# safes/RayTracing-Weekend

Hardware: AMD Instinct MI355X
Metric: Msamples/s, Cornell box 1920x1080 4096spp (higher is better)
Workload: dtype f32

## Files before the change

### raytracing_weekend_amd/csrc/rtw_hip.hip

```cpp
#include <hip/hip_runtime.h>

#include <algorithm>
#include <cmath>
#include <cstdio>
#include <cstdlib>
#include <cstring>
#include <condition_variable>
#include <exception>
#include <mutex>
#include <new>
#include <stdexcept>
#include <string>
#include <thread>
#include <vector>

#include "../../include/rtw.h"
#include "rtw_bvh.h"
#include "rtw_device.h"
#include "rtw_plan.h"
#include "rtw_kernels.h"
#include "rtw_guides.h"
#include "rtw_adaptive.h"
#ifndef RTW_SPLIT_BUILD
#include "rtw_guides.hip"
// ... 795 lines not shown
    }
    const unsigned pix_grid = pixel_grid(c, npix);
    for (const PathPass& ps : plan.passes) {
        HIP_TRY(c, hipMemsetAsync(c->d_queue, 0, 4, s));
        HIP_TRY(c, hipMemsetAsync(c->d_queue + 4, 0, 4, s));
        hipEvent_t ev_a = nullptr, ev_b = nullptr;
        HIP_TRY(c, log.event(ev_a));
        HIP_TRY(c, log.event(ev_b));
        HIP_TRY(c, hipEventRecord(ev_a, s));
        CallLog::Timed tp;
        HIP_TRY(c, log.open(tp, RTW_K_PATH, s));
        for (int part = 0; part < 2; part++) {
            const PathLaunch& l = ps.part[part];
            if (l.count == 0) continue;
            KArgs a = base;
            a.stats = c->d_stats;
            a.sample0 = (uint32_t)P->sample_offset;
            a.queue = c->d_queue + (part == 0 ? 0 : 4);
            a.order = c->d_order;
            a.order_counts = c->d_queue + 1;
            a.blocksum = c->blocksum + (part == 0 ? 0 : ps.slots_coarse) * npix;
            a.unit_sums = (part == 0 && plan.unit_sums) ? 1u : 0u;
            a.n_jobs = (uint32_t)l.n_jobs; a.n_ranges = (uint32_t)l.n_ranges; a.units_per_job = (uint32_t)l.jb;
            a.block0 = (uint32_t)(ps.b0 + l.first); a.n_blocks_pass = (uint32_t)l.count; a.unit_blocks = (uint32_t)l.unit_blocks;
            hipStream_t ls = part == 0 ? s : c->stream2;
            if (part == 1) HIP_TRY(c, hipStreamWaitEvent(ls, ev_a, 0));
            launch(RTW_K_PATH, P->rng_kind, a, l.grid, 0, ls);
            log.launches++;
            if (part == 1) {
                HIP_TRY(c, hipEventRecord(ev_b, ls));
                HIP_TRY(c, hipStreamWaitEvent(s, ev_b, 0));
            }
        }
        HIP_TRY(c, log.close(tp, s));
        if (plan.unit_sums)
            hipLaunchKernelGGL(k_resolve_blocks, dim3(pix_grid), dim3(kBlock), 0, s, (const float4*)c->blocksum, c->accum, (uint32_t)npix, (uint32_t)ps.slots_coarse,
                               (uint32_t)(ps.nb - ps.nb_coarse), (uint32_t)(ps.b0 + ps.nb_coarse));
        else
            hipLaunchKernelGGL(k_resolve_blocks, dim3(pix_grid), dim3(kBlock), 0, s, (const float4*)c->blocksum, c->accum, (uint32_t)npix, 0u, (uint32_t)ps.nb, (uint32_t)ps.b0);
    }
    hipLaunchKernelGGL(k_finish, dim3(pix_grid), dim3(kBlock), 0, s, (const float4*)c->accum, (const float4*)nullptr, (const float4*)nullptr, out, (uint32_t)npix, (float)P->spp);
    return RTW_OK;
}

int issue_batch(rtw_ctx* c, const WavefrontPlan& w, const Tuning& tune, KArgs a, rtw_ctx::Lane& L, size_t paths, size_t Sb, hipEvent_t ready,
                CallLog& log, bool list) {
    const size_t lds = c->lds_bytes;
    const uint32_t regions = w.grid_for(paths);
    HIP_TRY(c, hipStreamWaitEvent(L.st, ready, 0));
    HIP_TRY(c, hipMemsetAsync(L.cnt, 0, (size_t)regions * (w.sched.size() + 2) * sizeof(uint32_t), L.st));
    a.lbuf = L.lbuf;
    a.stats = c->d_stats;
    a.n_regions = regions;
    a.n_paths = (uint32_t)paths;
    a.region_cap = (uint32_t)w.cap_for(paths);
    a.trace_first = w.split_first ? 1u : 0u;
    a.first_group_log2 = 0;
    while (a.first_group_log2 < (uint32_t)tune.first_group_log2 && (Sb >> (a.first_group_log2 + 1)) << (a.first_group_log2 + 1) == Sb) a.first_group_log2++;
    int cur = 0;
    size_t ci = 0;
    a.out = L.buf[0];
    a.hit_out = L.hit[0];
    a.cnt_out = L.cnt;
    a.depth = 0; a.n_iter = 1;
    log.launches++;
    HIP_TRY(c, log.launch(L.st, RTW_K_FIRST, a, (int)regions, c->sc.use_bvh ? (size_t)(kBlock / 64) * (size_t)c->stack_depth * sizeof(uint32_t) : 0, kBlock, list));
    for (const Step& st : w.sched) {
        a.in = L.buf[cur];
        a.hit = L.hit[cur];
        a.hit_out = L.hit[cur];
        a.cnt_in = L.cnt + ci * regions;
        a.depth = (uint32_t)st.depth;
        a.n_iter = (uint32_t)st.n_iter;
        if (st.kind == RTW_K_TRACE) {
            if (c->sc.use_bvh) {
                KArgs at = a;
                at.sc.n_lds_nodes = w.trace_nodes; at.sc.n_lds_leaves = w.trace_leaves;
                HIP_TRY(c, log.launch(L.st, RTW_K_TRACE, at, w.trace_grid, w.trace_lds, w.trace_block));
            } else {
                HIP_TRY(c, log.launch(L.st, RTW_K_TRACE, a, (int)regions, lds));
            }
        } else {
            a.out = L.buf[cur ^ 1];
            a.hit_out = L.hit[cur ^ 1];
            a.cnt_out = L.cnt + (ci + 1) * regions;
            HIP_TRY(c, log.launch(L.st, st.kind, a, (int)regions, st.kind == RTW_K_BOUNCE ? lds : 0));
            cur ^= 1;
            ci++;
        }
        log.launches++;
    }
    return RTW_OK;
}

int render_wavefront(rtw_ctx* c, const rtw_params* P, const Tuning& tune, const KArgs& base, float4* out, hipStream_t s, CallLog& log) {
    const size_t npix = base.npix;
    const SceneFacts sf{c->sc.use_bvh != 0, c->sc.n_vol, c->n_tree_nodes, c->n_tree_leaves, c->stack_depth, c->sc.stack_wide != 0};
    WavefrontPlan w;
    for (;;) {
        w = plan_wavefront(tune, npix, P->spp, P->samples_per_pass, P->max_depth, c->pool_cap, c->n_cu, sf);
        if (w.trace_lds > 48 * 1024) {
            DScene ts = c->sc;
            ts.n_lds_nodes = w.trace_nodes;
            const void* f = (const void*)trace_bvh_kernel(w.trace_block, trace_bvh_mode(ts));
            HIP_TRY(c, hipFuncSetAttribute(f, hipFuncAttributeMaxDynamicSharedMemorySize, (int)w.trace_lds));
        }
        const int rc = ensure_pool(c, w.n_lanes, (size_t)w.regions_max * w.region_cap_max, npix, w.cnt_words, c->sc.n_lights > 0);
        if (rc == RTW_OK) break;
        if (rc != RTW_ERR_OOM || P->samples_per_pass > 0 || w.S <= 1) return rc;
        free_pool(c);
        (void)hipGetLastError();
        c->pool_cap = std::max<size_t>((size_t)tune.lanes * npix, npix * w.S * (size_t)tune.lanes / 2);
    }

    HIP_TRY(c, hipEventRecord(log.begin, s));
    HIP_TRY(c, hipMemsetAsync(c->accum, 0, npix * sizeof(float4), s));
    HIP_TRY(c, hipMemsetAsync(c->part, 0, npix * sizeof(float4), s));
    HIP_TRY(c, hipMemsetAsync(c->upart, 0, npix * sizeof(float4), s));
    HIP_TRY(c, hipMemsetAsync(c->d_stats, 0, (kStatRows + 1) * 8 * sizeof(unsigned long long), s));
    const unsigned pix_grid = pixel_grid(c, npix);
    hipEvent_t ev_ready = nullptr;
    if (P->max_depth > 0) {
        HIP_TRY(c, log.event(ev_ready));
        HIP_TRY(c, hipEventRecord(ev_ready, s));
    }
    for (size_t s0 = 0, b = 0; P->max_depth > 0 && s0 < (size_t)P->spp; b++) {
        const size_t Sb = w.batch_size(b, s0);
        rtw_ctx::Lane& L = c->lane[b % (size_t)w.n_lanes];
        KArgs a = base;
        a.sample0 = (uint32_t)(P->sample_offset + (int)s0);
        const int rc = issue_batch(c, w, tune, a, L, npix * Sb, Sb, b < (size_t)w.n_lanes ? ev_ready : L.ev_free, log, false);
        if (rc) return rc;
        HIP_TRY(c, hipEventRecord(L.ev_done, L.st));
        HIP_TRY(c, hipStreamWaitEvent(s, L.ev_done, 0));
        hipLaunchKernelGGL(k_resolve, dim3(pix_grid), dim3(kBlock), 0, s, (const float4*)L.lbuf, c->accum, c->upart, c->part, (uint32_t)npix, (uint32_t)Sb, (uint32_t)s0);
        HIP_TRY(c, hipEventRecord(L.ev_free, s));
        s0 += Sb;
    }
    hipLaunchKernelGGL(k_finish, dim3(pix_grid), dim3(kBlock), 0, s, (const float4*)c->accum, (const float4*)c->upart, (const float4*)c->part, out, (uint32_t)npix, (float)P->spp);
    return RTW_OK;
}

int print_diagnostics(rtw_ctx* c, bool path, const unsigned long long* hs) {
#ifdef RTW_PHASE_TIMERS
    if (path) {
        unsigned long long ph[8];
        HIP_TRY(c, hipMemcpy(ph, c->d_stats + kStatRows * 8, sizeof ph, hipMemcpyDeviceToHost));
        double tot = 0;
        for (int q = 0; q < 6; q++) tot += (double)ph[q];
        const char* nm[6] = {"refill", "regen", "walk_r", "shade_a", "walk_s", "shade_b"};
        fprintf(stderr, "[rtw] k_path wave-cycles by phase:");
        for (int q = 0; q < 6; q++) fprintf(stderr, " %s %.1f%%", nm[q], 100.0 * (double)ph[q] / tot);
        fprintf(stderr, " (total %.3g wave-cycles, %.0f per 64 segments)\n", tot, tot / ((double)hs[0] / 64.0));
    }
#endif
#ifdef RTW_SUBPHASE_TIMERS
    if (path) {
        static std::vector<unsigned long long> tab((size_t)kSubWaves * kSubRows);
        HIP_TRY(c, hipMemcpyFromSymbol(tab.data(), HIP_SYMBOL(g_sub_cyc), tab.size() * sizeof(unsigned long long)));
        double sum[kSubRows] = {0};
        for (size_t w = 0; w < (size_t)kSubWaves; w++) for (int q = 0; q < 14; q++) sum[q] += (double)tab[w * kSubRows + q];
        double tot = 0;
        for (int q = 0; q < 14; q++) tot += sum[q];
        const char* nm[9] = {"outside", "hitrec+philox", "lambert", "light", "metal", "diel", "iso", "nee", "entry"};
        fprintf(stderr, "[rtw] k_path wave-cycles by sub-phase of the closest-hit program:");
        for (int q = 0; q < 9; q++) fprintf(stderr, " %s %.1f%%", nm[q], 100.0 * sum[q] / tot);
        fprintf(stderr, " (total %.3g)\n", tot);
        std::fill(tab.begin(), tab.end(), 0ull);
        HIP_TRY(c, hipMemcpyToSymbol(HIP_SYMBOL(g_sub_cyc), tab.data(), tab.size() * sizeof(unsigned long long)));
    }
#endif
#ifdef RTW_TRACE_COUNT
    {
        unsigned long long w[7];
        HIP_TRY(c, hipMemcpy(w, c->d_stats + kStatRows * 8, sizeof w, hipMemcpyDeviceToHost));
        const double rays = (double)w[6];
        fprintf(stderr, "[rtw] k_trace_bvh: rays %.4g; per ray: node visits %.2f, primitive tests %.2f; wave steps per 64 rays: inner %.2f (lanes busy %.2f), leaf %.2f (lanes busy %.2f), outer %.2f\n",
                rays, (double)hs[6] / rays, (double)hs[7] / rays, (double)w[0] * 64.0 / rays, (double)hs[6] / ((double)w[0] * 64.0), (double)w[1] * 64.0 / rays,
                (double)hs[7] / ((double)w[1] * 64.0), (double)hs[2 + RTW_K_BOUNCE] * 64.0 / rays);
        const double tt = (double)(w[2] + w[3] + w[4] + w[5]);
        fprintf(stderr, "[rtw] k_trace_bvh wave-cycles: refill %.1f%% inner %.1f%% leaf %.1f%% finish %.1f%% (%.0f per 64 rays; per inner wave step %.0f, per leaf wave step %.0f)\n",
                100.0 * (double)w[2] / tt, 100.0 * (double)w[3] / tt, 100.0 * (double)w[4] / tt, 100.0 * (double)w[5] / tt, tt * 64.0 / rays,
                (double)w[3] / (double)w[0], (double)w[4] / (double)w[1]);
    }
#endif
    (void)c; (void)path; (void)hs;
    return RTW_OK;
}

KArgs render_args(const rtw_ctx* c, const rtw_params* P, size_t npix) {
    KArgs base = shard_args(c->sc, P, npix);
    if (P->estimator != RTW_EST_REFERENCE) {
        base.sc.estimator = P->estimator; base.sc.has_tex = P->estimator == RTW_EST_MIXTURE ? 2 : 1;
        base.sc.ray_tmin = 1.0e-3f; base.sc.probe_eps = 1.0e-3f;
    }
    return base;
}
bool path_pipeline(const rtw_ctx* c, const rtw_params* P, const Tuning& tune) {
    const bool path_small = !c->sc.use_bvh && c->sc.n_prims <= kPathMaxPrims && (c->sc.n_walk_words > 0 || c->sc.has_tex);
    const bool fits16 = P->width <= 65535 && P->height <= 65535;
    return P->max_depth > 0 && tune.path != 0 && fits16 && path_small;
}

int render_single(rtw_ctx* c, const rtw_params* P, void* d_rgba, hipStream_t s, rtw_stats* stats) {
    HIP_TRY(c, hipSetDevice(c->device));
    if (!s) s = c->stream;
    const size_t npix = shard_rows(P) * (size_t)P->width;
    if (stats) memset(stats, 0, sizeof *stats);
    if (npix == 0) return RTW_OK;
    if (npix > 0xffffffffull / 2) return fail(c, RTW_ERR_UNSUPPORTED, "tile too large");

    const Tuning tune = read_tuning();
    CallLog log{c, P->rng_kind, stats != nullptr && tune.kernel_timing};
    HIP_TRY(c, log.event(log.begin));
    HIP_TRY(c, log.event(log.end));
    const KArgs base = render_args(c, P, npix);
    const bool use_path = path_pipeline(c, P, tune);
    int rc = use_path ? render_path(c, P, tune, base, (float4*)d_rgba, s, log) : render_wavefront(c, P, tune, base, (float4*)d_rgba, s, log);
    if (rc) return rc;
    HIP_TRY(c, hipGetLastError());
    HIP_TRY(c, hipEventRecord(log.end, s));
    HIP_TRY(c, hipEventSynchronize(log.end));

    unsigned long long hs[8] = {0, 0, 0, 0, 0, 0, 0, 0};
    {
        unsigned long long rows_[kStatRows * 8];
        HIP_TRY(c, hipMemcpy(rows_, c->d_stats, sizeof rows_, hipMemcpyDeviceToHost));
        for (uint32_t r = 0; r < kStatRows; r++)
            for (int k = 0; k < 8; k++) hs[k] += rows_[r * 8 + k];
    }
    rc = print_diagnostics(c, use_path, hs);
    if (rc) return rc;
    if (stats) {
        float ms = 0.f;
        HIP_TRY(c, hipEventElapsedTime(&ms, log.begin, log.end));
        stats->seconds = (double)ms * 1e-3;
        stats->bounce_seconds = stats->seconds;
        for (const CallLog::Timed& t : log.timed) {
            float m = 0.f;
            HIP_TRY(c, hipEventElapsedTime(&m, t.a, t.b));
            stats->kernel_seconds[t.kind] += (double)m * 1e-3;
            stats->kernel_launches[t.kind]++;
        }
        for (int k = 0; k < RTW_K_COUNT; k++) stats->kernel_segments[k] = hs[2 + k];
        stats->bounce_launches = log.launches;
        stats->samples = (uint64_t)npix * (uint64_t)P->spp;
        stats->segments = hs[0];
        stats->shadow_rays = hs[1];
        stats->algorithmic_bytes = 128ull * stats->segments + 32ull * stats->samples;
    }
    return RTW_OK;
}

__global__ void __launch_bounds__(256) k_interleave(const float4* __restrict__ stage, float4* __restrict__ out, uint32_t width, uint32_t rows, uint32_t n,
                                                    const uint32_t* __restrict__ shard_off) {
    const size_t total = (size_t)rows * width;
    for (size_t i = (size_t)blockIdx.x * blockDim.x + threadIdx.x; i < total; i += (size_t)gridDim.x * blockDim.x) {
        const uint32_t r = (uint32_t)(i / width), x = (uint32_t)(i - (size_t)r * width);
        const uint32_t g = r % n, l = r / n;
        out[i] = stage[((size_t)shard_off[g] + l) * width + x];
    }
}

int run_shard(rtw_ctx* kc, Worker& w) {
    test_fault("worker");
    if (hipSetDevice(kc->device) != hipSuccess) return fail(kc, RTW_ERR_DEVICE, "hipSetDevice failed");
    if (w.npix == 0) return RTW_OK;
    if (w.npix > kc->out_pix) {
        if (kc->d_out) (void)hipFree(kc->d_out);
        kc->d_out = nullptr; kc->out_pix = 0;
        if (hipMalloc(&kc->d_out, w.npix * sizeof(float4)) != hipSuccess) return fail(kc, RTW_ERR_OOM, "shard buffer");
        kc->out_pix = w.npix;
    }
    const int rc = render_single(kc, &w.P, kc->d_out, nullptr, w.want_stats ? &w.st : nullptr);
    if (rc) return rc;
    HIP_TRY(kc, hipMemcpyPeerAsync(w.gather_dst, w.gather_dev, kc->d_out, kc->device, w.npix * sizeof(float4), kc->stream));
    HIP_TRY(kc, hipStreamSynchronize(kc->stream));
    return RTW_OK;
}
void worker_main(rtw_ctx* kc) {
    Worker& w = *kc->worker;
    for (;;) {
        try {
            std::unique_lock<std::mutex> lk(w.m);
            w.cv.wait(lk, [&] { return w.has_job || w.quit; });
            if (w.quit) return;
            lk.unlock();
            int rc;
            try {
                rc = run_shard(kc, w);
            } catch (const std::bad_alloc&) {
                rc = fail_nothrow(kc, RTW_ERR_OOM, "out of host memory in a worker thread (std::bad_alloc)");
            } catch (const std::exception& e) {
                rc = fail_nothrow(kc, RTW_ERR_DEVICE, e.what());
            } catch (...) {
                rc = fail_nothrow(kc, RTW_ERR_DEVICE, "unknown exception in a worker thread");
            }
            lk.lock();
            w.rc = rc; w.has_job = false; w.done = true;
            lk.unlock();
            w.cv.notify_all();
        } catch (...) {
            w.rc = RTW_ERR_DEVICE; w.has_job = false; w.done = true;
            w.cv.notify_all();
            return;
        }
// ... 551 lines not shown
```

### raytracing_weekend_amd/csrc/rtw_kernels.h

```cpp
#pragma once
#include "rtw_device.h"
#include "rtw_plan.h"

namespace rtwk {
using namespace rtwdev;

#ifndef RTW_MIN_WAVES
#define RTW_MIN_WAVES 1
#endif
#ifdef RTW_SUBPHASE_TIMERS
constexpr int kSubRows = 16, kSubWaves = 8192;
__device__ unsigned long long g_sub_cyc[kSubWaves][kSubRows];
RTW_DEV constexpr int rtw_sub_id(const char* n) {
    return n[0] != 's' || n[1] != 'a' ? 0 : n[3] == 'h' ? 1 : n[3] == 'l' && n[4] == 'a' ? 2 : n[3] == 'l' ? 3 : n[3] == 'm' ? 4 : n[3] == 'd' ? 5 : n[3] == 'i' ? 6 : n[3] == 'n' ? 7 : 0;
}
RTW_DEV void rtw_sub_stamp(int id) {
    const unsigned long long t_in = __builtin_amdgcn_s_memtime();
    if ((threadIdx.x & 63u) == 0u) {
        unsigned long long* row = g_sub_cyc[(blockIdx.x * (blockDim.x >> 6) + (threadIdx.x >> 6)) % kSubWaves];
        const unsigned long long open_id = row[14], t0 = row[15];
        if (t0 != 0ull) row[open_id] += t_in - t0;
        row[14] = (unsigned long long)id;
        __builtin_amdgcn_s_waitcnt(0);
        row[15] = __builtin_amdgcn_s_memtime();
// ... 983 lines not shown
                        fogged = volume_pass<Rng<KIND>, true>(A.sc, so, nee.dir, nee.tmin, 0.0f, gt, g, tv, pv);
                    }
                    if (fogged) nee.has = false;
                    else { p.ldir = nee.dir; p.ltmax = nee.tmax; p.c = vmul(nee.rad, p.T); }
                }
                const bool alive = shade_b<KIND>(A.depth, A.max_depth, g, ev, so, sd, att, radiance, p.o, p.d, p.T, p.L, TEX == 2 && A.sc.estimator == RTW_EST_MIXTURE);
                if (ev == EV_HIT) p.o = so;
                p.a = g.a; p.b = g.b;
                if (alive) {
                    p.ray_time = (KIND == RTW_RNG_TEA_LCG || A.sc.has_motion) ? g.ray_time(A.depth + 1u) : 0.0f;
                    p.b = g.b;
                    keep = true;
                } else if (nee.has) {
                    p.gk |= kZombie;
                    keep = true;
                } else {
                    finish_path(A, path_id_of<KIND>(A, p), p.L);
                }
            }
        }
        compact_store(A, s_cursor, keep, p);
    }
    cursor_publish(A, s_cursor, n_seg, n_shadow, RTW_K_SHADE);
}

template <int KIND, int TEX>
__global__ void __launch_bounds__(kBlock, RTW_MIN_WAVES) k_bounce(const KArgs A) {
    extern __shared__ uint32_t s_stack[];
    RTW_WORKLIST_SHARED
    RTW_CURSOR_SHARED
    RTW_NOISE_SHARED
    const uint32_t tid = threadIdx.x;
    cursor_init(s_cursor);
    const uint32_t* noise_lds = stage_noise<(TEX != 0)>(A.sc, s_noise);
    const TravMem tm = trav_mem(A.sc, s_stack, kBlock, tid);
    uint32_t n_seg = 0, n_shadow = 0;
    const WorkList wl = worklist_init(A.cnt_in, A.n_regions, s_pref, s_part);
    for (uint32_t vc = blockIdx.x; vc < wl.total_chunks; vc += gridDim.x) {
        uint32_t region, chunk, n_valid;
        worklist_lookup(wl, A.n_regions, vc, region, chunk, n_valid);
        const uint32_t idx = chunk * kBlock + tid;
        const bool valid = tid < n_valid;
        bool keep = false;
        Path p;
        p.gk = 0; p.ltmax = -1.f;
        if (valid) {
            load_path(A.in, (size_t)region * A.region_cap + idx, p, A.sc.n_lights > 0);
            Rng<KIND> g;
            rng_from_path<KIND>(g, A.seed, p);
            const float gt = gather_time_of(A, p.gk);
            if (p.ltmax >= 0.0f) {
                float st;
                int sprim;
                traverse<Rng<KIND>, true, true>(A.sc, p.o, p.ldir, A.sc.probe_eps, p.ltmax, 0.0f, gt, g, tm, st, sprim);
                if (sprim < 0) p.L = vadd(p.L, p.c);
                p.ltmax = -1.0f;
            }
            if (p.gk & kZombie) {
                finish_path(A, path_id_of<KIND>(A, p), p.L);
            } else {
                uint32_t depth = A.depth;
                bool alive = false;
                uint32_t nee_prev = (p.gk & kNeePrev) ? 1u : 0u;
                for (uint32_t it = 0; it < A.n_iter; it++) {
                    float t;
                    int prim;
                    traverse<Rng<KIND>, false, false>(A.sc, p.o, p.d, A.sc.ray_tmin, 1.e27f, p.ray_time, gt, g, tm, t, prim);
                    v3 so, sd, att, radiance;
                    Nee nee;
                    const int ev = shade_a<KIND, TEX>(A.sc, g, p.o, p.d, gt, t, prim, so, sd, att, radiance, nee, noise_lds, nee_prev);
                    n_seg++;
                    if (nee.has) {
                        float st;
                        int sprim;
                        traverse<Rng<KIND>, true, false>(A.sc, so, nee.dir, nee.tmin, nee.tmax, 0.0f, gt, g, tm, st, sprim);
                        n_shadow++;
                        if (sprim < 0) radiance = vadd(radiance, nee.rad);
                    }
                    alive = shade_b<KIND>(depth, A.max_depth, g, ev, so, sd, att, radiance, p.o, p.d, p.T, p.L, TEX == 2 && A.sc.estimator == RTW_EST_MIXTURE);
                    depth++;
                    if (!alive) break;
                    p.ray_time = (KIND == RTW_RNG_TEA_LCG || A.sc.has_motion) ? g.ray_time(depth) : 0.0f;
                }
                p.a = g.a; p.b = g.b;
                p.gk = (p.gk & ~kNeePrev) | (nee_prev ? kNeePrev : 0u);
                if (alive) keep = true;
                else finish_path(A, path_id_of<KIND>(A, p), p.L);
            }
        }
        compact_store(A, s_cursor, keep, p);
    }
    cursor_publish(A, s_cursor, n_seg, n_shadow, RTW_K_BOUNCE);
}

RTW_DEV uint32_t order_lookup(const KArgs& A, uint32_t gi) {
    const uint32_t n_groups = (A.npix + 63u) / 64u;
    const uint32_t c2 = A.order_counts[0], c1 = A.order_counts[1];
    const uint32_t idx = gi < c2 ? gi : (gi < c2 + c1 ? n_groups + (gi - c2) : 2u * n_groups + (gi - c2 - c1));
    return __builtin_amdgcn_readfirstlane(A.order[idx]);
}

template <bool WALK>
__global__ void __launch_bounds__(kBlock) k_classify(const KArgs A, uint32_t* __restrict__ order, uint32_t* __restrict__ counters, uint32_t n_groups) {
    __shared__ u32x4 s_walk[WALK ? kWalkMaxWords : 1];
    if (WALK) {
        for (uint32_t i = threadIdx.x; i < (uint32_t)A.sc.n_walk_words; i += kBlock) s_walk[i] = A.sc.walk[i];
        __syncthreads();
    }
    const uint32_t lane = threadIdx.x & 63u;
    const uint32_t waves = gridDim.x * (kBlock / 64u);
    for (uint32_t g = blockIdx.x * (kBlock / 64u) + (threadIdx.x >> 6); g < n_groups; g += waves) {
        const uint32_t p_local = g * 64u + lane;
        bool may = false, specular = false;
        if (p_local < A.npix) {
            const uint32_t yl = fastdiv(p_local, A.divw_m, A.divw_s1, A.divw_s2);
            const uint32_t x = p_local - yl * A.width, y = A.row0 + yl * A.row_stride;
            const rtw_camera& cam = A.sc.cam;
            if (A.sc.cam_type != RTW_CAM_PERSPECTIVE || cam.lens_radius != 0.0f) {
                may = true;
            } else {
                const float s = ((float)x + 0.5f) / (float)A.width, t = ((float)y + 0.5f) / (float)A.height;
                const v3 o = ld3(cam.origin);
                const v3 d = vsub(vfma(ld3(cam.vertical), t, vfma(ld3(cam.horizontal), s, ld3(cam.lower_left))), o);
                may = may_hit_scene(A.sc, o, d);
                if (WALK && may) {
                    float th;
                    int prim;
                    walk_lds<false>(s_walk, A.sc.n_groups, o, d, A.sc.ray_tmin, 1.e27f, th, prim);
                    if (prim >= 0) {
                        const int mt = A.sc.hitrec[prim].mat_type;
                        specular = mt == RTW_MAT_METAL || mt == RTW_MAT_DIELECTRIC;
                    }
                }
            }
        }
        const bool any = __ballot(may) != 0ull;
        const uint32_t n_spec = (uint32_t)__popcll(__ballot(specular));
        if (lane == 0) {
            const uint32_t cls = !any ? 0u : (n_spec >= 16u ? 2u : 1u);
            order[(2u - cls) * n_groups + atomicAdd(&counters[2u - cls], 1u)] = g;
        }
    }
}

#if defined(RTW_PHASE_TIMERS)
#define RTW_MARK(name) { const unsigned long long now_ = __builtin_amdgcn_s_memtime(); ph_cyc[ph_cur] += now_ - ph_t0; ph_t0 = now_; ph_cur = rtw_phase_id(name); }
RTW_DEV constexpr int rtw_phase_id(const char* n) { return n[0] == 'r' && n[2] == 'f' ? 0 : n[0] == 'r' ? 1 : n[0] == 'w' && n[5] == 'r' ? 2 : n[0] == 's' && n[6] == 'a' ? 3 : n[0] == 'w' ? 4 : 5; }
#else
#define RTW_MARK(name) asm volatile("; MARK " name)
#endif
#ifndef RTW_PATH_WAVES
#define RTW_PATH_WAVES 5
#endif
#ifndef RTW_PATH_COLD_WAVES
#define RTW_PATH_COLD_WAVES RTW_MIN_WAVES
#endif
template <int KIND, int TEX, int MEDIA5 = 0, int LIST = 0>
__global__ void __launch_bounds__(kBlock, TEX ? (MEDIA5 ? 5 : RTW_PATH_COLD_WAVES) : RTW_PATH_WAVES) k_path(const KArgs A) {
    RTW_NOISE_SHARED
    __shared__ u32x4 s_hitrec[kPathMaxPrims * 6];
    const uint32_t tid = threadIdx.x;
    const uint32_t* noise_lds = stage_noise<(TEX != 0)>(A.sc, s_noise);
    {
        const u32x4* src = (const u32x4*)A.sc.hitrec;
        for (uint32_t i = tid; i < (uint32_t)A.sc.n_prims * 6u; i += kBlock) s_hitrec[i] = src[i];
    }
    __shared__ float s_usum[3][kBlock];
    __shared__ PathConsts s_pc;
    if (tid == 0) {
        for (int q = 0; q < 3; q++) {
            s_pc.cam_o[q] = A.sc.cam.origin[q]; s_pc.cam_ll[q] = A.sc.cam.lower_left[q];
            s_pc.cam_h[q] = A.sc.cam.horizontal[q]; s_pc.cam_v[q] = A.sc.cam.vertical[q];
        }
        for (int q = 0; q < 5; q++) s_pc.rect[q] = A.sc.pdf.rect[q];
        int gen = A.sc.pdf.gen;
        if (gen == RTW_PDF_MIXTURE || gen == RTW_PDF_MIXTURE_BIAS) gen = A.sc.pdf.p1_gen;
        s_pc.gen = gen;
        if (A.sc.n_lights > 0) {
            for (int q = 0; q < 3; q++) { s_pc.lnrm[q] = A.sc.lights[0].normal[q]; s_pc.lemi[q] = A.sc.lights[0].emission[q]; }
            s_pc.larea = A.sc.lights[0].area;
        }
        s_pc.npix = LIST ? A.order[0] : A.npix; s_pc.width = A.width; s_pc.row0 = A.row0; s_pc.row_stride = A.row_stride;
        s_pc.divs_m = A.divs_m; s_pc.divs_s1 = A.divs_s1; s_pc.divs_s2 = A.divs_s2; s_pc.spp = A.spp;
        s_pc.bs_lo = (uint32_t)(uint64_t)A.blocksum; s_pc.bs_hi = (uint32_t)((uint64_t)A.blocksum >> 32);
        s_pc.unit_shift = (A.unit_sums && !LIST) ? 3u : 0u; s_pc.list_lo = LIST ? (uint32_t)(uint64_t)(A.order + 1) : 0u;
        s_pc.n_jobs = A.n_jobs; s_pc.n_ranges = A.n_ranges; s_pc.units_per_job = A.units_per_job; s_pc.unit_blocks = A.unit_blocks;
        s_pc.n_blocks_pass = A.n_blocks_pass; s_pc.block0 = A.block0; s_pc.divw_m = A.divw_m; s_pc.divw_s1 = A.divw_s1; s_pc.divw_s2 = A.divw_s2;
        s_pc.q_lo = (uint32_t)(uint64_t)A.queue; s_pc.q_hi = (uint32_t)((uint64_t)A.queue >> 32); s_pc.list_hi = LIST ? (uint32_t)((uint64_t)(A.order + 1) >> 32) : 0u;
    }
    const PathConsts* pc_cam = TEX ? nullptr : &s_pc;
    __shared__ u32x4 s_walk[TEX ? 1 : kWalkMaxWords];
    if (!TEX) for (uint32_t i = tid; i < (uint32_t)A.sc.n_walk_words; i += kBlock) s_walk[i] = A.sc.walk[i];
    __syncthreads();
    const uint32_t lane = tid & 63u;
    uint32_t u_next = 0, u_end = 0, job_g = 0, job_b = 0;
    bool exhausted = false;
    bool need = true;
    uint32_t pxy = 0, blk = 0, blk_end = 0, s_cur = 0;
    v3 usum = V(0.f, 0.f, 0.f);
    bool alive = false;
    uint32_t depth = 0, rng_a = 0;
    uint32_t gk = 0, rng_b = 0, nee_prev = 0;
    float ray_time = 0.f;
    v3 o = V(0.f, 0.f, 0.f), d = o, T = o, L = o;
    uint32_t n_seg = 0, n_shadow = 0;
#ifdef RTW_PHASE_TIMERS
    unsigned long long ph_cyc[6] = {0, 0, 0, 0, 0, 0}, ph_t0 = __builtin_amdgcn_s_memtime();
    int ph_cur = 0;
#endif
    for (;;) {
        RTW_MARK("refill");
        unsigned long long need_mask = __ballot(need);
        while (need_mask != 0ull && !exhausted) {
            const PathConsts* kc = &s_pc;
            if (u_next >= u_end) {
                uint32_t q = 0;
                if (lane == 0) q = atomicAdd((uint32_t*)(((uint64_t)kc->q_hi << 32) | kc->q_lo), 1u);
                q = __builtin_amdgcn_readfirstlane(q);
                if (q >= (uint32_t)__builtin_amdgcn_readfirstlane((int)kc->n_jobs)) { exhausted = true; break; }
                const uint32_t n_ranges = (uint32_t)__builtin_amdgcn_readfirstlane((int)kc->n_ranges), upj = (uint32_t)__builtin_amdgcn_readfirstlane((int)kc->units_per_job);
                const uint32_t gi = q / n_ranges;
                job_g = LIST ? gi : order_lookup(A, gi);
                job_b = (q - gi * n_ranges) * upj;
                u_next = 0; u_end = 64u * upj;
                continue;
            }
            const uint32_t avail = u_end - u_next;
            const uint32_t rank = __builtin_amdgcn_mbcnt_hi((uint32_t)(need_mask >> 32), __builtin_amdgcn_mbcnt_lo((uint32_t)need_mask, 0u));
            if (need && rank < avail) {
                const uint32_t ub = kc->unit_blocks, nbp = kc->n_blocks_pass;
                const uint32_t u = u_next + rank;
                const uint32_t b = (job_b + (u >> 6)) * ub;
                const uint32_t p_local = job_g * 64u + (u & 63u);
                if (p_local < kc->npix && b < nbp) {
                    need = false;
                    blk = b;
                    blk_end = min(b + ub, nbp);
                    uint32_t pix = p_local;
                    if (LIST) {
                        pix = ((const uint32_t*)(((uint64_t)kc->list_hi << 32) | kc->list_lo))[p_local];
                        s_usum[0][tid] = __uint_as_float(p_local);
                    }
                    const uint32_t yl = fastdiv(pix, kc->divw_m, kc->divw_s1, kc->divw_s2);
                    pxy = (pix - yl * kc->width) | ((kc->row0 + yl * kc->row_stride) << 16);
                    s_cur = (kc->block0 + b) * kSumBlock;
                    usum = V(0.f, 0.f, 0.f);
                    alive = false;
                }
            }
            u_next += min((uint32_t)__popcll(need_mask), avail);
            need_mask = __ballot(need);
        }
        if (__ballot(!need) == 0ull) break;
        RTW_MARK("regen");
        const bool busy = !need;
        const uint32_t px = pxy & 0xffffu, py = pxy >> 16;
        Rng<KIND> g;
        if (busy && !alive) {
            Path p;
            raygen<KIND, !TEX>(A, px, py, A.sample0 + s_cur, 0u, p, g, pc_cam);
            o = p.o; d = p.d; T = p.T; L = p.L; rng_a = p.a;
            if (TEX) { ray_time = p.ray_time; gk = p.gk; rng_b = p.b; nee_prev = 0; }
            depth = 0; alive = true;
        }
        if (busy) {
            const uint32_t pixel = A.width * py + px;
            if (KIND == RTW_RNG_TEA_LCG) g.init(A.seed, 0, 0, rng_a, rng_b);
            else g.init(A.seed, pixel, A.sample0 + s_cur, rng_a, A.sample0 + s_cur);
        }
        RTW_MARK("walk_r");
        const float gt = TEX ? gather_time_of(A, gk) : 0.0f;
        float th = 1.e27f;
        int prim = -1;
        const bool walk = busy && (depth > 0u || may_hit_scene(A.sc, o, d));
        if (__ballot(walk) != 0ull) {
            if (busy) {
                if (TEX) traverse_brute<Rng<KIND>, false, false>(A.sc, o, d, A.sc.ray_tmin, 1.e27f, ray_time, gt, g, th, prim);
                else walk_lds<false>(s_walk, A.sc.n_groups, o, d, A.sc.ray_tmin, 1.e27f, th, prim);
            }
        }
        RTW_MARK("shade_a");
#ifdef RTW_SUBPHASE_TIMERS
        rtw_sub_stamp(8);
#endif
        if (busy) {
            v3 so, sd, att, radiance;
            Nee nee;
            const int ev = shade_a<KIND, TEX>(A.sc, g, o, d, gt, th, prim, so, sd, att, radiance, nee, noise_lds, nee_prev, s_hitrec, &s_pc);
            n_seg++;
#ifdef RTW_SUBPHASE_TIMERS
            rtw_sub_stamp(0);
#endif
            RTW_MARK("walk_s");
            if (nee.has) {
                float st;
                int sprim;
                if (TEX) traverse_brute<Rng<KIND>, true, false>(A.sc, so, nee.dir, nee.tmin, nee.tmax, 0.0f, gt, g, st, sprim);
                else walk_lds<true>(s_walk, A.sc.n_groups, so, nee.dir, nee.tmin, nee.tmax, st, sprim);
                n_shadow++;
                if (sprim < 0) radiance = vadd(radiance, nee.rad);
            }
            RTW_MARK("shade_b");
            alive = shade_b<KIND>(depth, A.max_depth, g, ev, so, sd, att, radiance, o, d, T, L, TEX == 2 && A.sc.estimator == RTW_EST_MIXTURE);
            depth++;
            rng_a = g.a;
            if (alive) {
                if (TEX) {
                    ray_time = (KIND == RTW_RNG_TEA_LCG || A.sc.has_motion) ? g.ray_time(depth) : 0.0f;
                    rng_b = g.b;
                }
            } else {
                usum = vadd(usum, V((L.x == L.x) ? L.x : 0.f, (L.y == L.y) ? L.y : 0.f, (L.z == L.z) ? L.z : 0.f));
                s_cur++;
                if ((s_cur % kSumBlock) == 0u || s_cur >= A.spp) {
                    const PathConsts* kc = &s_pc;
                    const uint32_t c_row0 = kc->row0, c_stride = kc->row_stride, c_width = kc->width, c_npix = kc->npix;
                    const uint32_t yl_ = c_stride > 1 ? fastdiv(py - c_row0, kc->divs_m, kc->divs_s1, kc->divs_s2) : py - c_row0;
                    const uint32_t pix = LIST ? __float_as_uint(s_usum[0][tid]) : yl_ * c_width + px;
                    const uint32_t b_done = blk;
                    blk++;
                    need = blk >= blk_end || s_cur >= A.spp;
                    float4* const bsum_base = (float4*)(((uint64_t)kc->bs_hi << 32) | kc->bs_lo);
                    const uint32_t ush = kc->unit_shift;
                    v3 prev = V(0.f, 0.f, 0.f);
                    if (ush != 0u && (b_done % kSumUnitBlocks) != 0u) prev = V(s_usum[0][tid], s_usum[1][tid], s_usum[2][tid]);
                    const v3 u = vadd(prev, usum);
                    if (ush == 0u || need || (blk % kSumUnitBlocks) == 0u) bsum_base[(size_t)(b_done >> ush) * c_npix + pix] = make_float4(u.x, u.y, u.z, 0.f);
                    else { s_usum[0][tid] = u.x; s_usum[1][tid] = u.y; s_usum[2][tid] = u.z; }
                    usum = V(0.f, 0.f, 0.f);
                }
            }
        }
    }
#ifdef RTW_PHASE_TIMERS
    RTW_MARK("refill");
    if (lane == 0) for (int q = 0; q < 6; q++) atomicAdd(&A.stats[kStatRows * 8 + q], ph_cyc[q]);
#endif
    for (int off = 32; off > 0; off >>= 1) {
        n_seg += __shfl_down(n_seg, off);
        n_shadow += __shfl_down(n_shadow, off);
    }
    if (lane == 0) {
        unsigned long long* row = stat_row(A);
        if (n_seg) { atomicAdd(&row[0], (unsigned long long)n_seg); atomicAdd(&row[2 + RTW_K_PATH], (unsigned long long)n_seg); }
        if (n_shadow) atomicAdd(&row[1], (unsigned long long)n_shadow);
    }
}

#ifndef RTW_TEMPLATES_ONLY
__global__ void __launch_bounds__(kBlock) k_resolve_blocks(const float4* __restrict__ slots, float4* __restrict__ accum, uint32_t npix, uint32_t n_unit_slots,
                                                           uint32_t n_block_slots, uint32_t first_block) {
    for (uint32_t i = blockIdx.x * blockDim.x + threadIdx.x; i < npix; i += gridDim.x * blockDim.x) {
        float4 a = accum[i];
        for (uint32_t u = 0; u < n_unit_slots; u++) {
            const float4 l = slots[(size_t)u * npix + i];
            a.x += l.x; a.y += l.y; a.z += l.z;
        }
        float ux = 0.f, uy = 0.f, uz = 0.f;
        for (uint32_t b = 0; b < n_block_slots; b++) {
            const float4 l = slots[(size_t)(n_unit_slots + b) * npix + i];
            ux += l.x; uy += l.y; uz += l.z;
            if (((first_block + b + 1u) % kSumUnitBlocks) == 0u || b + 1u == n_block_slots) {
                a.x += ux; a.y += uy; a.z += uz;
                ux = 0.f; uy = 0.f; uz = 0.f;
            }
        }
        accum[i] = a;
    }
}

__global__ void __launch_bounds__(kBlock) k_atrous(const float4* __restrict__ in, float4* __restrict__ out, int width, int height, int step, float inv_sigma2) {
    const int n = width * height;
    for (int i = blockIdx.x * blockDim.x + threadIdx.x; i < n; i += gridDim.x * blockDim.x) {
        const int y = i / width, x = i - y * width;
        const float4 c = in[i];
        const float kern[5] = {1.0f / 16.0f, 1.0f / 4.0f, 3.0f / 8.0f, 1.0f / 4.0f, 1.0f / 16.0f};
        float sr = 0.f, sg = 0.f, sb = 0.f, sw = 0.f;
        for (int dy = -2; dy <= 2; dy++) {
            int yy = y + dy * step;
            yy = yy < 0 ? 0 : (yy > height - 1 ? height - 1 : yy);
            for (int dx = -2; dx <= 2; dx++) {
                int xx = x + dx * step;
                xx = xx < 0 ? 0 : (xx > width - 1 ? width - 1 : xx);
                const float4 q = in[yy * width + xx];
                const float dr = c.x - q.x, dg = c.y - q.y, db = c.z - q.z;
                const float d2 = (dr * dr + dg * dg) + db * db;
                const float w = (kern[dy + 2] * kern[dx + 2]) / (1.0f + d2 * inv_sigma2);
                sr = sr + w * q.x; sg = sg + w * q.y; sb = sb + w * q.z; sw = sw + w;
            }
        }
        out[i] = make_float4(sr / sw, sg / sw, sb / sw, c.w);
    }
}

__global__ void __launch_bounds__(kBlock) k_resolve(const float4* __restrict__ lbuf, float4* __restrict__ accum, float4* __restrict__ upart, float4* __restrict__ part,
                                                    uint32_t npix, uint32_t nslots, uint32_t first_sample) {
    for (uint32_t i = blockIdx.x * blockDim.x + threadIdx.x; i < npix; i += gridDim.x * blockDim.x) {
        float4 a = accum[i], u = upart[i], b = part[i];
        for (uint32_t s = 0; s < nslots; s++) {
            const uint32_t rel = first_sample + s;
            if (rel != 0u && (rel % kSumBlock) == 0u) {
                u.x += b.x; u.y += b.y; u.z += b.z;
                b = make_float4(0.f, 0.f, 0.f, 0.f);
                if ((rel % (kSumBlock * kSumUnitBlocks)) == 0u) {
                    a.x += u.x; a.y += u.y; a.z += u.z;
                    u = make_float4(0.f, 0.f, 0.f, 0.f);
                }
            }
            float4 l = lbuf[(size_t)s * npix + i];
            b.x += l.x; b.y += l.y; b.z += l.z;
        }
        accum[i] = a;
        upart[i] = u;
        part[i] = b;
    }
}

__global__ void __launch_bounds__(kBlock) k_finish(const float4* __restrict__ accum, const float4* __restrict__ upart, const float4* __restrict__ part,
                                                   float4* __restrict__ out, uint32_t npix, float spp) {
    for (uint32_t i = blockIdx.x * blockDim.x + threadIdx.x; i < npix; i += gridDim.x * blockDim.x) {
        float4 a = accum[i];
        if (part != nullptr) {
            float4 u = upart[i];
            const float4 b = part[i];
            u.x += b.x; u.y += b.y; u.z += b.z;
            a.x += u.x; a.y += u.y; a.z += u.z;
        }
        out[i] = make_float4(a.x / spp, a.y / spp, a.z / spp, 1.0f);
    }
}

__global__ void __launch_bounds__(kBlock) k_debug_intersect(const DScene sc, const float* __restrict__ rays, const float* __restrict__ ray_time,
                                                           const float* __restrict__ gather_time, int n, float* __restrict__ out_t,
                                                           int32_t* __restrict__ out_prim, uint32_t stack_stride) {
    extern __shared__ uint32_t s_stack[];
    const TravMem tm = trav_mem(sc, s_stack, stack_stride, threadIdx.x);
    int i = blockIdx.x * blockDim.x + threadIdx.x;
    if (i >= n) return;
    const float* r = rays + 8 * (size_t)i;
    NoRng g;
    float t;
    int prim;
    traverse<NoRng, false, true>(sc, V(r[0], r[1], r[2]), V(r[3], r[4], r[5]), r[6], r[7], ray_time ? ray_time[i] : 0.f,
                                 gather_time ? gather_time[i] : 0.f, g, tm, t, prim);
    out_t[i] = t;
    out_prim[i] = prim;
}

__global__ void __launch_bounds__(kBlock) k_debug_math(int op, unsigned long long* __restrict__ tally) {
    const uint32_t T = gridDim.x * blockDim.x;
    uint32_t differ = 0, fast = 0, first = 0xffffffffu;
    for (uint64_t p = blockIdx.x * blockDim.x + threadIdx.x; p < (1ull << 32); p += T) {
        const uint32_t bits = (uint32_t)p;
        const float x = __uint_as_float(bits);
        float want, got;
        bool in;
        if (op == 0) {
            want = 1.0f / x; in = rtwmath::rcp_window(x); got = rtwmath::rcp_short<MathHw>(x);
        } else if (op == 1) {
            want = __builtin_sqrtf(x); in = rtwmath::sqrt_window(x); got = rtwmath::sqrt_short<MathHw>(x);
        } else if (op == 2) {
            want = 1.0f / __builtin_sqrtf(x); in = rtwmath::sqrt_window(x); got = rtwmath::rcp_sqrt_short<MathHw>(x);
        } else if (op == 3) {
            want = 1.0f / x; in = rtwmath::rcp_window(x); got = rtwmath::rcp_short<MathHw, 1>(x);
        } else if (op == 4) {
            want = 1.0f / x; in = rtwmath::rcp_window(x); got = rtwmath::rcp_short<MathHw, 2>(x);
        } else if (op == 5) {
            want = __builtin_sqrtf(x); in = rtwmath::sqrt_window(x); got = rtwmath::sqrt_short<MathHw, 0>(x);
        } else {
            want = __builtin_sqrtf(x); in = rtwmath::sqrt_window(x); got = rtwmath::sqrt_short<MathHw, 1>(x);
        }
        if (!in) continue;
        fast++;
        const bool same = __float_as_uint(got) == __float_as_uint(want) || (got != got && want != want);
        if (!same) { differ++; first = bits < first ? bits : first; }
    }
    atomicAdd(&tally[1], (unsigned long long)fast);
    if (differ) { atomicAdd(&tally[0], (unsigned long long)differ); atomicMin(&tally[2], (unsigned long long)first); }
}

#endif

}
```

Measured before the change: 17370.

## Pre-generate camera rays ahead into LDS to amortize divergent raygen

When any lane in a wave needs a new camera ray, the other busy lanes also generate directions for their upcoming samples and stash them in a per-thread LDS ring of depth RTW_REGEN_AHEAD. Later restarts pop a stored direction instead of running raygen, which is meant to cut the number of wave iterations that pay for divergent raygen. It assumes a pinhole camera with the origin from shared constants, unit throughput and zero rng_a, and it adds LDS use that could lower occupancy. Phase timers also gain counters for loop iterations and raygen iterations.

```diff
diff --git a/raytracing_weekend_amd/csrc/rtw_hip.hip b/raytracing_weekend_amd/csrc/rtw_hip.hip
--- a/raytracing_weekend_amd/csrc/rtw_hip.hip
+++ b/raytracing_weekend_amd/csrc/rtw_hip.hip
@@ -971,6 +971,8 @@
         fprintf(stderr, "[rtw] k_path wave-cycles by phase:");
         for (int q = 0; q < 6; q++) fprintf(stderr, " %s %.1f%%", nm[q], 100.0 * (double)ph[q] / tot);
         fprintf(stderr, " (total %.3g wave-cycles, %.0f per 64 segments)\n", tot, tot / ((double)hs[0] / 64.0));
+        fprintf(stderr, "[rtw] k_path loop iterations %.4g, lane utilisation %.3f, iterations that ran raygen %.3f\n", (double)ph[6],
+                (double)hs[0] / (64.0 * (double)ph[6]), (double)ph[7] / (double)ph[6]);
     }
 #endif
 #ifdef RTW_SUBPHASE_TIMERS
diff --git a/raytracing_weekend_amd/csrc/rtw_kernels.h b/raytracing_weekend_amd/csrc/rtw_kernels.h
--- a/raytracing_weekend_amd/csrc/rtw_kernels.h
+++ b/raytracing_weekend_amd/csrc/rtw_kernels.h
@@ -1159,6 +1159,9 @@
 #ifndef RTW_PATH_WAVES
 #define RTW_PATH_WAVES 5
 #endif
+#ifndef RTW_REGEN_AHEAD
+#define RTW_REGEN_AHEAD 2
+#endif
 #ifndef RTW_PATH_COLD_WAVES
 #define RTW_PATH_COLD_WAVES RTW_MIN_WAVES
 #endif
@@ -1207,6 +1210,11 @@
     v3 usum = V(0.f, 0.f, 0.f);
     bool alive = false;
     uint32_t depth = 0, rng_a = 0;
+    constexpr bool AHEAD = RTW_REGEN_AHEAD && !TEX && KIND == RTW_RNG_PHILOX;
+    constexpr uint32_t kAhead = AHEAD ? RTW_REGEN_AHEAD : 1;
+    static_assert((kAhead & (kAhead - 1u)) == 0u, "RTW_REGEN_AHEAD: 0 or a power of two");
+    __shared__ float s_ahead[kAhead][AHEAD ? 3 : 1][AHEAD ? kBlock : 1];
+    uint32_t n_ahead = 0;
     uint32_t gk = 0, rng_b = 0, nee_prev = 0;
     float ray_time = 0.f;
     v3 o = V(0.f, 0.f, 0.f), d = o, T = o, L = o;
@@ -1214,8 +1222,12 @@
 #ifdef RTW_PHASE_TIMERS
     unsigned long long ph_cyc[6] = {0, 0, 0, 0, 0, 0}, ph_t0 = __builtin_amdgcn_s_memtime();
     int ph_cur = 0;
+    unsigned long long n_iter = 0, n_regen = 0;
 #endif
     for (;;) {
+#ifdef RTW_PHASE_TIMERS
+        n_iter++;
+#endif
         RTW_MARK("refill");
         unsigned long long need_mask = __ballot(need);
         while (need_mask != 0ull && !exhausted) {
@@ -1253,6 +1265,7 @@
                     s_cur = (kc->block0 + b) * kSumBlock;
                     usum = V(0.f, 0.f, 0.f);
                     alive = false;
+                    n_ahead = 0;
                 }
             }
             u_next += min((uint32_t)__popcll(need_mask), avail);
@@ -1263,7 +1276,38 @@
         const bool busy = !need;
         const uint32_t px = pxy & 0xffffu, py = pxy >> 16;
         Rng<KIND> g;
-        if (busy && !alive) {
+        if (AHEAD) {
+            const bool want = busy && !alive;
+            const bool take = want && n_ahead > 0u;
+            if (take) {
+                const uint32_t sl = s_cur & (kAhead - 1u);
+                d = V(s_ahead[sl][0][tid], s_ahead[sl][1][tid], s_ahead[sl][2][tid]);
+                n_ahead--;
+            }
+            const bool now = want && !take;
+            if (__ballot(now) != 0ull) {
+#ifdef RTW_PHASE_TIMERS
+                n_regen++;
+#endif
+                const uint32_t s_gen = now ? s_cur : s_cur + 1u + n_ahead;
+                const bool fill = busy && !now && n_ahead < kAhead && s_gen < A.spp && blk + (s_gen / kSumBlock - s_cur / kSumBlock) < blk_end;
+                if (now || fill) {
+                    Path p;
+                    Rng<KIND> g_cam;
+                    raygen<KIND, true>(A, px, py, A.sample0 + s_gen, 0u, p, g_cam, pc_cam);
+                    if (now) d = p.d;
+                    else {
+                        const uint32_t sl = s_gen & (kAhead - 1u);
+                        s_ahead[sl][0][tid] = p.d.x; s_ahead[sl][1][tid] = p.d.y; s_ahead[sl][2][tid] = p.d.z;
+                        n_ahead++;
+                    }
+                }
+            }
+            if (want) {
+                o = ld3(s_pc.cam_o); T = V(1.f, 1.f, 1.f); L = V(0.f, 0.f, 0.f); rng_a = 0u;
+                depth = 0; alive = true;
+            }
+        } else if (busy && !alive) {
             Path p;
             raygen<KIND, !TEX>(A, px, py, A.sample0 + s_cur, 0u, p, g, pc_cam);
             o = p.o; d = p.d; T = p.T; L = p.L; rng_a = p.a;
@@ -1342,6 +1386,7 @@
 #ifdef RTW_PHASE_TIMERS
     RTW_MARK("refill");
     if (lane == 0) for (int q = 0; q < 6; q++) atomicAdd(&A.stats[kStatRows * 8 + q], ph_cyc[q]);
+    if (lane == 0) { atomicAdd(&A.stats[kStatRows * 8 + 6], n_iter); atomicAdd(&A.stats[kStatRows * 8 + 7], n_regen); }
 #endif
     for (int off = 32; off > 0; off >>= 1) {
         n_seg += __shfl_down(n_seg, off);
```

Result: no change. 17530 (median of 6 runs) (+0.9%).
